# NVlabs/nvbio

Measured on NVIDIA H100. Metric: Mreads/s (150bp) seed+extend, higher is better.
Workload: dtype int32

## Files before the change

### nvbio_b200/csrc/pipeline.cu

```cuda
#include "fm_core.cuh"
#include "gotoh_core.cuh"
#include "pipeline_core.cuh"
#include "gotoh_full_core.cuh"
#include <cub/agent/single_pass_scan_operators.cuh>
#include <cub/block/block_scan.cuh>
#include <cub/device/device_scan.cuh>
#include <cub/device/device_segmented_sort.cuh>
#include <mutex>

namespace nvb {

struct PipeGeom {
    uint32_t n_reads;
    uint32_t n_strings;
    uint32_t strands;
    uint32_t stride;
    uint32_t bits;
    uint32_t seeds_per_string;
    uint32_t seed_len, seed_interval;
    uint32_t band;
    uint32_t max_seed_hits;
    uint32_t genome_len;
};

template <int BITS>
__global__ void __launch_bounds__(256)
pipe_make_strings_kernel(const StrSet reads, const PipeGeom g, uint32_t* __restrict__ out_words, uint32_t* __restrict__ out_len)
{
    constexpr uint32_t SPW = 32 / BITS;
    const uint32_t words_per_string = g.stride / SPW;
    const uint64_t t = (uint64_t)blockIdx.x * 256 + threadIdx.x;
    if (t >= (uint64_t)g.n_strings * words_per_string) return;
    const uint32_t s = (uint32_t)(t / words_per_string), w = (uint32_t)(t % words_per_string);
    const uint32_t read = s / g.strands, strand = s % g.strands;
    const uint32_t off = str_off(reads, read), len = str_len(reads, read);
    if (w == 0) out_len[s] = len;
    uint32_t word = 0;
    for (uint32_t k = 0; k < SPW; ++k) {
        const uint32_t p = w * SPW + k;
        uint32_t c = 0;
        if (p < len) {
            if (strand == 0) c = sym_at_rt(reads.words, reads.bits, reads.big_endian, off + p);
            else { c = sym_at_rt(reads.words, reads.bits, reads.big_endian, off + (len - 1u - p)); c = (c < 4u) ? 3u - c : c; }
        }
        word |= c << (32u - BITS - BITS * k);
    }
    out_words[t] = word;
}

__global__ void __launch_bounds__(256)
pipe_make_quals_kernel(const StrSet reads, const PipeGeom g, const uint8_t* __restrict__ quals, uint8_t* __restrict__ out)
{
    const uint64_t t = (uint64_t)blockIdx.x * 256 + threadIdx.x;
    if (t >= (uint64_t)g.n_strings * g.stride) return;
    const uint32_t s = (uint32_t)(t / g.stride), p = (uint32_t)(t % g.stride);
    const uint32_t read = s / g.strands, strand = s % g.strands;
// ... 130 lines not shown
        ranges[q] = make_uint2(x, y);
        if (sizes) sizes[q] = seed_range_hits(make_uint2(x, y), g.max_seed_hits);
    }
}

__device__ __forceinline__ uint32_t upper_bound_u32(const uint32_t* __restrict__ a, uint32_t n, uint32_t v)
{
    uint32_t lo = 0, hi = n;
    while (lo < hi) { const uint32_t mid = (lo + hi) >> 1; if (a[mid] <= v) lo = mid + 1; else hi = mid; }
    return lo;
}

__global__ void pipe_count_kernel(const uint32_t* __restrict__ excl, const uint32_t* __restrict__ sizes, uint32_t n_queries, uint32_t capacity,
                                  uint32_t* __restrict__ counts)
{
    if (threadIdx.x == 0 && blockIdx.x == 0) {
        const uint32_t total = n_queries ? excl[n_queries - 1] + sizes[n_queries - 1] : 0u;
        counts[1] = total;
        counts[0] = total < capacity ? total : capacity;
    }
}

__global__ void __launch_bounds__(256)
pipe_expand_hits_kernel(const FmIndex f, const PipeGeom g, const uint2* __restrict__ ranges, const uint32_t* __restrict__ sizes,
                        const uint32_t* __restrict__ excl, const uint32_t* __restrict__ slen, const uint32_t* __restrict__ counts,
                        uint32_t* __restrict__ hit_string, uint32_t* __restrict__ p_off, uint32_t* __restrict__ p_len,
                        uint32_t* __restrict__ t_off, uint32_t* __restrict__ t_len)
{
    const uint32_t q = blockIdx.x * 256 + threadIdx.x;
    if (q >= g.n_strings * g.seeds_per_string) return;
    const uint32_t sz = sizes[q];
    if (sz == 0) return;
    const uint32_t base = excl[q], kept = counts[0];
    const uint32_t x = ranges[q].x;
    const uint32_t s = q / g.seeds_per_string, k = q % g.seeds_per_string;
    const uint32_t seed_begin = k * g.seed_interval;
    const uint32_t len = slen[s];
    for (uint32_t j = 0; j < sz; ++j) {
        const uint32_t h = base + j;
        if (h >= kept) break;
        const uint2 w = hit_window(fm_locate_one(f, x + j), seed_begin, len, g);
        hit_string[h] = s;
        p_off[h] = s * g.stride; p_len[h] = len;
        t_off[h] = w.x;          t_len[h] = w.y - w.x;
    }
}

struct Jobs { uint32_t *p_off, *p_len, *t_off, *t_len; };

constexpr uint32_t RJ_BLOCK = 128;
constexpr uint32_t RJ_STAGE = 640;
constexpr int      RJ_LOCAL = 6;
constexpr uint32_t RJ_CLAIMED = 0xFFFFFFFFu, RJ_CLAIMED_EMPTY = 0xFFFFFFFEu;
using RjTileState = cub::ScanTileState<uint32_t>;
using RjPrefixOp  = cub::TilePrefixCallbackOp<uint32_t, ::cuda::std::plus<uint32_t>, RjTileState>;

__global__ void __launch_bounds__(256)
pipe_resolve_init_kernel(RjTileState tiles, const uint32_t n_tiles, uint32_t* __restrict__ counts, uint32_t* __restrict__ dp_count)
{
    tiles.InitializeStatus((int)n_tiles);
    if (blockIdx.x == 0 && threadIdx.x == 0) { counts[2] = 0u; counts[3] = 0u; *dp_count = 0u; }
}

__global__ void __launch_bounds__(RJ_BLOCK, 8)
pipe_resolve_reads_kernel(const FmIndex f, const PipeGeom g, const uint2* __restrict__ ranges, const uint32_t* __restrict__ slen,
                          const uint32_t hit_capacity, RjTileState tiles, const uint32_t n_tiles, uint32_t* __restrict__ counts,
                          const int shortcut, const int32_t match, const int32_t mismatch, const int32_t max_gap_open,
                          const uint32_t* __restrict__ str_words, const uint32_t* __restrict__ genome,
                          uint32_t* __restrict__ j_string, uint32_t* __restrict__ j_first, const Jobs jobs,
                          int32_t* __restrict__ job_score, uint2* __restrict__ job_sink,
                          const Jobs dp, uint32_t* __restrict__ dp_job, uint32_t* __restrict__ dp_count,
                          unsigned long long* __restrict__ best_key, int32_t* best_score, uint32_t* best_pos, uint8_t* __restrict__ best_strand)
{
    using BlockScan = cub::BlockScan<uint32_t, RJ_BLOCK>;
    __shared__ struct { typename RjPrefixOp::TempStorage prefix; typename BlockScan::TempStorage scan; } s_tmp;
    __shared__ uint32_t st_string[RJ_STAGE], st_first[RJ_STAGE], st_toff[RJ_STAGE], st_tlen[RJ_STAGE], st_slot[RJ_STAGE];
    __shared__ unsigned long long s_key[RJ_BLOCK];
    __shared__ int32_t s_score[RJ_BLOCK];
    __shared__ uint32_t s_pos[RJ_BLOCK];
    __shared__ uint8_t s_strand[RJ_BLOCK];
    __shared__ uint32_t s_tile, s_cnt, s_base, s_dp_cnt, s_dp_base;
    if (threadIdx.x == 0) { s_tile = atomicAdd(counts + 3, 1u); s_cnt = 0u; s_dp_cnt = 0u; }
    s_key[threadIdx.x] = 0ull;
    __syncthreads();
    const uint32_t tile = s_tile, r0 = tile * RJ_BLOCK, r = r0 + threadIdx.x;
    const uint32_t per_read = g.strands * g.seeds_per_string;
    const bool live = r < g.n_reads;
    const uint2* rr = ranges + (size_t)r * per_read;

    uint32_t hits = 0, run = 0;
    if (live)
        for (uint32_t q = 0; q < per_read; ++q) hits += seed_range_hits(rr[q], g.max_seed_hits);
    if (tile == 0) {
        uint32_t aggregate;
        BlockScan(s_tmp.scan).ExclusiveSum(hits, run, aggregate);
        if (threadIdx.x == 0) tiles.SetInclusive(0, aggregate);
    } else {
        RjPrefixOp prefix(tiles, s_tmp.prefix, ::cuda::std::plus<uint32_t>{}, (int)tile);
        BlockScan(s_tmp.scan).ExclusiveSum(hits, run, prefix);
    }
    if (tile == n_tiles - 1u && threadIdx.x == RJ_BLOCK - 1u) {
        const uint32_t total = run + hits;
        counts[1] = total;
        counts[0] = total < hit_capacity ? total : hit_capacity;
    }

    if (live) {
        uint32_t lk_s[RJ_LOCAL], lk_b[RJ_LOCAL], lk_e[RJ_LOCAL];
        int n_local = 0;
        for (uint32_t strand = 0; strand < g.strands; ++strand) {
            const uint32_t s = r * g.strands + strand;
            const uint32_t len = slen[s];
            for (uint32_t k = 0; k < g.seeds_per_string; ++k) {
                const uint2 rq = rr[strand * g.seeds_per_string + k];
                const bool located = rq.y == 0xFFFFFFFFu;
                const uint32_t sz = seed_range_hits(rq, g.max_seed_hits);
                if (sz == 0u) continue;
                const uint32_t base = run, x = rq.x, seed_begin = k * g.seed_interval;
                run += sz;
                for (uint32_t j = 0; j < sz; ++j) {
                    const uint32_t h = base + j;
                    if (h >= hit_capacity) break;
                    const uint2 w = hit_window(located ? x : fm_locate_one(f, x + j), seed_begin, len, g);
                    bool seen = false;
#pragma unroll
                    for (int e = 0; e < RJ_LOCAL; ++e) seen |= (e < n_local) && lk_s[e] == s && lk_b[e] == w.x && lk_e[e] == w.y;
                    if (seen) continue;
#pragma unroll
                    for (int e = 0; e < RJ_LOCAL; ++e) if (e == n_local) { lk_s[e] = s; lk_b[e] = w.x; lk_e[e] = w.y; }
                    if (n_local < RJ_LOCAL) ++n_local;
                    const uint32_t slot = atomicAdd(&s_cnt, 1u);
                    if (slot < RJ_STAGE) { st_string[slot] = s; st_first[slot] = h; st_toff[slot] = w.x; st_tlen[slot] = w.y - w.x; }
                    else {
                        const uint32_t o = atomicAdd(counts + 2, 1u), d = atomicAdd(dp_count, 1u);
                        j_string[o] = s; j_first[o] = h;
                        jobs.p_off[o] = s * g.stride; jobs.p_len[o] = len; jobs.t_off[o] = w.x; jobs.t_len[o] = w.y - w.x;
                        dp.p_off[d] = s * g.stride; dp.p_len[d] = len; dp.t_off[d] = w.x; dp.t_len[d] = w.y - w.x; dp_job[d] = o;
                    }
                }
            }
        }
    }
    __syncthreads();

    const uint32_t n = s_cnt < RJ_STAGE ? s_cnt : RJ_STAGE;
    if (threadIdx.x == 0) s_base = n ? atomicAdd(counts + 2, n) : 0u;
    __syncthreads();
    for (uint32_t i = threadIdx.x; i < n; i += RJ_BLOCK) {
        const uint32_t o = s_base + i, s = st_string[i], first = st_first[i], len = slen[s], to = st_toff[i], N = st_tlen[i];
        j_string[o] = s; j_first[o] = first; jobs.p_off[o] = s * g.stride; jobs.p_len[o] = len; jobs.t_off[o] = to; jobs.t_len[o] = N;
        int32_t score = 0; uint32_t sx = 0, sy = 0;
        if (shortcut && gapless_job_shortcut(str_words, genome, s * g.stride, len, to, N, g.band, match, mismatch, max_gap_open, score, sx, sy,
                                             shortcut != 2)) {
            const uint2 sk = make_uint2(sx, sy);
            job_score[o] = score; job_sink[o] = sk;
            if (job_aligned(sk)) {
                st_slot[i] = RJ_CLAIMED; st_toff[i] = to + sx; st_tlen[i] = (uint32_t)score;
                atomicMax(&s_key[s / g.strands - r0], make_best_key(score, first));
            } else st_slot[i] = RJ_CLAIMED_EMPTY;
        } else st_slot[i] = atomicAdd(&s_dp_cnt, 1u);
    }
    __syncthreads();
    if (threadIdx.x == 0) s_dp_base = s_dp_cnt ? atomicAdd(dp_count, s_dp_cnt) : 0u;
    __syncthreads();
    for (uint32_t i = threadIdx.x; i < n; i += RJ_BLOCK) {
        const uint32_t slot = st_slot[i], s = st_string[i];
        if (slot == RJ_CLAIMED) {
            const uint32_t rl = s / g.strands - r0;
            const int32_t score = (int32_t)st_tlen[i];
            if (s_key[rl] == make_best_key(score, st_first[i])) { s_score[rl] = score; s_pos[rl] = st_toff[i]; s_strand[rl] = (uint8_t)(s % g.strands); }
        } else if (slot != RJ_CLAIMED_EMPTY) {
            const uint32_t d = s_dp_base + slot;
            dp.p_off[d] = s * g.stride; dp.p_len[d] = slen[s]; dp.t_off[d] = st_toff[i]; dp.t_len[d] = st_tlen[i]; dp_job[d] = s_base + i;
        }
    }
    __syncthreads();
    if (live) {
        const unsigned long long key = s_key[threadIdx.x];
        best_key[r] = key;
        best_score[r] = key ? s_score[threadIdx.x] : INT_MIN;
        best_pos[r] = key ? s_pos[threadIdx.x] : 0xFFFFFFFFu;
        best_strand[r] = key ? s_strand[threadIdx.x] : (uint8_t)0;
    }
}

__global__ void __launch_bounds__(256)
pipe_scatter_dp_kernel(const PipeGeom g, const uint32_t* __restrict__ dp_count, const uint32_t* __restrict__ dp_job,
                       const int32_t* __restrict__ dp_score, const uint2* __restrict__ dp_sink,
                       const uint32_t* __restrict__ j_string, const uint32_t* __restrict__ j_first,
                       int32_t* __restrict__ job_score, uint2* __restrict__ job_sink, unsigned long long* __restrict__ best_key)
{
    const uint32_t n = *dp_count;
    for (uint32_t a = blockIdx.x * 256 + threadIdx.x; a < n; a += gridDim.x * 256) {
        const uint32_t j = dp_job[a];
        const int32_t sc = dp_score[a];
        const uint2 sk = dp_sink[a];
        job_score[j] = sc; job_sink[j] = sk;
        if (job_aligned(sk)) atomicMax(best_key + j_string[j] / g.strands, make_best_key(sc, j_first[j]));
    }
}

__global__ void __launch_bounds__(256)
pipe_finalize_dp_kernel(const PipeGeom g, const uint32_t* __restrict__ dp_count, const uint32_t* __restrict__ dp_job,
                        const int32_t* __restrict__ dp_score, const uint2* __restrict__ dp_sink, const uint32_t* __restrict__ dp_t_off,
                        const uint32_t* __restrict__ j_string, const uint32_t* __restrict__ j_first,
                        const unsigned long long* __restrict__ best_key,
// ... 898 lines not shown
    if (nq64 > 0x7FFFFFFFull) return NVB_E_UNSUPPORTED;
    if (nq64 * (uint64_t)P->max_seed_hits > 0xFFFFFFFFull) return NVB_E_UNSUPPORTED;

    const cudaStream_t s = c.s = as_stream(stream);
    c.P = P; c.f = make_fmindex(fmi); c.rd = make_strset(reads); c.genome = d_genome; c.nq = (uint32_t)nq64; c.hit_capacity = hit_capacity;
    c.best_score = d_best_score; c.best_pos = d_best_pos; c.hit_score = d_hit_score; c.hit_sink = d_hit_sink; c.BA = BA; c.PP = PP; c.PO = PO; c.MP = MP; c.MO = MO;
    if (PMO) {
        c.PMO = PMO;
        c.se_mo.d_second_score = PMO->d_mate_second_score; c.se_mo.d_mapq = PMO->d_mate_mapq;
        c.MO = &c.se_mo;
    }
    c.dedup = P->dedup_jobs != 0;
    c.per_read = c.dedup && g_pipe_path != 1 && !d_hit_read && !d_hit_window && !d_hit_score && !d_hit_sink;
    const nvb_gotoh_scheme& SC = P->scheme;
    c.eligible = c.per_read && P->type == NVB_LOCAL && g.bits == 2 && P->band_len <= 32 && !SC.d_qual_table && SC.match > 0 && SC.mismatch < 0 &&
                 SC.pattern_gap_open < 0 && SC.pattern_gap_ext <= 0 && SC.text_gap_open < 0 && SC.text_gap_ext <= 0;
    c.seed_split = c.per_read && c.f.sa_shift == 0u && c.f.ktab_k && g.seed_len > c.f.ktab_k && g_seed_split;
    size_t need = 0;
    NVB_TRY(c.carve(d_temp, need));
    if (!d_temp || *temp_bytes < need) { *temp_bytes = need; return NVB_E_TEMP_SIZE; }
    if (n_reads == 0) return NVB_OK;

    NVB_TRY(default_stage_events(&c.SE));
    NVB_TRY(c.stage(0));
    NVB_TRY(c.make_strings()); NVB_TRY(c.stage(1));
    NVB_TRY(c.match_seeds());  NVB_TRY(c.stage(2));
    if (!c.per_read) {
        size_t scan_bytes = c.scan_bytes;
        NVB_CUDA_TRY(cub::DeviceScan::ExclusiveSum(c.scan_tmp, scan_bytes, c.sizes, c.excl, (int)c.nq, s));
        pipe_count_kernel<<<1, 32, 0, s>>>(c.excl, c.sizes, c.nq, hit_capacity, c.counts);
        NVB_LAUNCH_CHECK();
    }
    NVB_TRY(c.stage(3));
    NVB_TRY(c.per_read ? c.extend_per_read() : c.extend_per_hit());
    if (hit_capacity && (d_hit_read || d_hit_window)) {
        pipe_export_hits_kernel<<<(hit_capacity + 255) / 256, 256, 0, s>>>(g, c.counts, c.hit_string, c.hits.t_off, c.hits.t_len, d_hit_read, (uint2*)d_hit_window);
        NVB_LAUNCH_CHECK();
    }
    if (BA && !PP) NVB_TRY(c.best_traceback());
    if (c.MO) NVB_TRY(c.second_best());
    if (PMO) NVB_TRY(c.pair_candidates());
    if (PP) NVB_TRY(c.paired_rescue());
    if (BA && PP) { NVB_TRY(c.best_traceback()); NVB_TRY(c.rescue_traceback()); }
    if (PMO) NVB_TRY(c.pair_second());
    if (!c.dedup) NVB_CUDA_TRY(cudaMemcpyAsync(c.counts + 2, c.counts, sizeof(uint32_t), cudaMemcpyDeviceToDevice, s));
    if (d_n_hits) NVB_CUDA_TRY(cudaMemcpyAsync(d_n_hits, c.counts, 3 * sizeof(uint32_t), cudaMemcpyDeviceToDevice, s));
    NVB_TRY(c.stage(7));
    c.SE->valid = true;
    return NVB_OK;
}

extern "C" void nvb_debug_pipeline_path(int path) { g_pipe_path = path; }
extern "C" void nvb_debug_seed_split(int on) { g_seed_split = on; }
extern "C" void nvb_debug_perfect_shortcut(int on) { g_perfect_shortcut = on; }
extern "C" int nvb_debug_dp_jobs(uint32_t* n)
{
    if (!n || !g_last_dp_count) return NVB_E_INVALID;
    NVB_CUDA_TRY(cudaDeviceSynchronize());
    NVB_CUDA_TRY(cudaMemcpy(n, g_last_dp_count, sizeof(uint32_t), cudaMemcpyDeviceToHost));
    return NVB_OK;
}

extern "C" int nvb_seed_extend(const nvb_fm_index* fmi, const uint32_t* d_genome,
                    const nvb_string_set* reads, uint32_t n_reads,
                    const nvb_seed_extend_params* P, uint32_t hit_capacity,
                    int32_t* d_best_score, uint32_t* d_best_pos,
                    uint32_t* d_n_hits, uint32_t* d_hit_read, nvb_uint2* d_hit_window,
                    int32_t* d_hit_score, nvb_uint2* d_hit_sink,
                    void* d_temp, size_t* temp_bytes, void* stream)
{
    return seed_extend_impl(fmi, d_genome, reads, n_reads, P, hit_capacity, d_best_score, d_best_pos, d_n_hits, d_hit_read, d_hit_window,
                            d_hit_score, d_hit_sink, nullptr, nullptr, nullptr, nullptr, nullptr, nullptr, d_temp, temp_bytes, stream);
}

extern "C" int nvb_seed_extend_traceback(const nvb_fm_index* fmi, const uint32_t* d_genome,
                    const nvb_string_set* reads, uint32_t n_reads,
                    const nvb_seed_extend_params* P, uint32_t hit_capacity,
                    int32_t* d_best_score, uint32_t* d_best_pos,
                    uint32_t* d_n_hits, uint32_t* d_hit_read, nvb_uint2* d_hit_window,
                    int32_t* d_hit_score, nvb_uint2* d_hit_sink,
                    const nvb_best_alignment_out* best_alignment,
                    void* d_temp, size_t* temp_bytes, void* stream)
{
    if (!best_alignment) return NVB_E_INVALID;
    return seed_extend_impl(fmi, d_genome, reads, n_reads, P, hit_capacity, d_best_score, d_best_pos, d_n_hits, d_hit_read, d_hit_window,
                            d_hit_score, d_hit_sink, best_alignment, nullptr, nullptr, nullptr, nullptr, nullptr, d_temp, temp_bytes, stream);
}

extern "C" int nvb_seed_extend_paired(const nvb_fm_index* fmi, const uint32_t* d_genome,
                    const nvb_string_set* reads, uint32_t n_pairs,
                    const nvb_seed_extend_params* P, uint32_t hit_capacity,
                    const nvb_pair_params* pair_params, const nvb_pair_out* out,
                    uint32_t* d_n_hits, void* d_temp, size_t* temp_bytes, void* stream)
{
    if (!pair_params || !out || n_pairs > 0x3FFFFFFFu || !temp_bytes) return NVB_E_INVALID;
    return seed_extend_impl(fmi, d_genome, reads, 2u * n_pairs, P, hit_capacity, out->d_mate_score, out->d_mate_pos, d_n_hits, nullptr, nullptr,
                            nullptr, nullptr, nullptr, pair_params, out, nullptr, nullptr, nullptr, d_temp, temp_bytes, stream);
}

extern "C" int nvb_seed_extend_mapq(const nvb_fm_index* fmi, const uint32_t* d_genome,
                    const nvb_string_set* reads, uint32_t n_reads,
                    const nvb_seed_extend_params* P, uint32_t hit_capacity,
                    int32_t* d_best_score, uint32_t* d_best_pos,
                    uint32_t* d_n_hits, uint32_t* d_hit_read, nvb_uint2* d_hit_window,
                    int32_t* d_hit_score, nvb_uint2* d_hit_sink,
                    const nvb_best_alignment_out* best_alignment,
                    const nvb_mapq_params* mapq, const nvb_mapq_out* mapq_out,
// ... 52 lines not shown
```

### nvbio_b200/csrc/pipeline_core.cuh

```cuda
#pragma once
#include "fm_core.cuh"

namespace nvb {

__host__ __device__ __forceinline__ uint32_t nvb_clz(uint32_t x) {
#ifdef __CUDA_ARCH__
    return (uint32_t)__clz((int)x);
#else
    return (uint32_t)__builtin_clz(x);
#endif
}

__host__ __device__ __forceinline__ uint32_t job_diff_bits(const uint32_t* __restrict__ str_words, const uint32_t* __restrict__ genome,
                                                           const uint32_t po, const uint32_t t, const uint32_t i, const uint32_t cnt)
{
    const uint32_t x = (be2_window(str_words, po + i, cnt) ^ be2_window(genome, t + i, cnt)) >> (32u - 2u * cnt);
    return (x | (x >> 1)) & 0x55555555u;
}
__host__ __device__ __forceinline__ uint32_t job_differences(const uint32_t* __restrict__ str_words, const uint32_t* __restrict__ genome,
                                                             const uint32_t po, const uint32_t M, const uint32_t t, const uint32_t limit)
{
    uint32_t mm = 0;
    for (uint32_t i = 0; i < M && mm <= limit; i += 16u) mm += nvb_popc(job_diff_bits(str_words, genome, po, t, i, M - i < 16u ? M - i : 16u));
    return mm;
}

__host__ __device__ __forceinline__ uint32_t diff_row_mask(const uint32_t w0, const uint32_t cnt, const uint32_t lo, const uint32_t hi)
{
    const uint32_t a = lo > w0 ? lo : w0, b = hi < w0 + cnt - 1u ? hi : w0 + cnt - 1u;
    if (a > b) return 0u;
    return ((2u << (2u * (w0 + cnt - 1u - a))) - 1u) & ~((1u << (2u * (w0 + cnt - 1u - b))) - 1u);
}
__host__ __device__ inline void job_diff_span(const uint32_t* __restrict__ str_words, const uint32_t* __restrict__ genome, const uint32_t po,
                                              const uint32_t t, const uint32_t lo, const uint32_t hi, int32_t& first, int32_t& last)
{
    first = (int32_t)hi + 1; last = (int32_t)lo - 1;
    for (uint32_t i = lo; i <= hi; i += 16u) {
        const uint32_t cnt = hi + 1u - i < 16u ? hi + 1u - i : 16u;
        const uint32_t d = job_diff_bits(str_words, genome, po, t, i, cnt);
        if (!d) continue;
        if (first > (int32_t)hi) first = (int32_t)(i + cnt - 1u - ((31u - nvb_clz(d)) >> 1));
        last = (int32_t)(i + cnt - 1u - ((31u - nvb_clz(d & (0u - d))) >> 1));
    }
}
__host__ __device__ __forceinline__ uint32_t text_window16(const uint32_t g0, const uint32_t g1, const uint32_t g2, const uint32_t g3, const uint32_t off)
{
    const uint32_t idx = off >> 4, sh = 2u * (off & 15u);
    const uint32_t hi = idx == 0u ? g0 : (idx == 1u ? g1 : g2), lo = idx == 0u ? g1 : (idx == 1u ? g2 : g3);
    return sh ? ((hi << sh) | (lo >> (32u - sh))) : hi;
}

__host__ __device__ inline bool gapless_job_shortcut(const uint32_t* __restrict__ str_words, const uint32_t* __restrict__ genome,
                                                     const uint32_t po, const uint32_t M, const uint32_t to, const uint32_t N, const uint32_t band,
                                                     const int32_t match, const int32_t mismatch, const int32_t max_gap_open,
                                                     int32_t& score, uint32_t& sink_x, uint32_t& sink_y, const bool one_gap = true)
{
    if (M < 1u || to == 0u || N < M + band - 1u) return false;
    const uint32_t j0 = band / 2u;
    const int32_t o = -max_gap_open, lim = !one_gap ? o : (o + match - mismatch < 2 * o ? o + match - mismatch : 2 * o);
    const uint32_t mm_max = (uint32_t)((lim - 1) / match);
    int32_t h = 0, best = 0, f1 = (int32_t)M, f2 = (int32_t)M, l1 = -1, l2 = -1; uint32_t end = 0, prev = 0, mm0 = 0;
    for (uint32_t i = 0; i < M && mm0 <= mm_max; i += 16u) {
        const uint32_t cnt = M - i < 16u ? M - i : 16u;
        uint32_t d = job_diff_bits(str_words, genome, po, to + j0, i, cnt);
        while (d && mm0 <= mm_max) {
            const uint32_t bit = 31u - nvb_clz(d);
            const uint32_t p = i + (cnt - 1u - (bit >> 1));
            d &= ~(1u << bit);
            h += match * (int32_t)(p - prev);
            if (h >= best) { best = h; end = p; }
            h += mismatch; h = h > 0 ? h : 0;
            if (mm0 == 0u) f1 = (int32_t)p; else if (mm0 == 1u) f2 = (int32_t)p;
            l2 = l1; l1 = (int32_t)p;
            prev = p + 1u; ++mm0;
        }
    }
    if (mm0 > mm_max) return false;
    h += match * (int32_t)(M - prev);
    if (h >= best) { best = h; end = M; }
    const int32_t delta = match * (int32_t)M - best;
    if (delta >= lim) return false;
    const bool gap1 = delta >= o;
    const uint32_t U = gap1 ? (uint32_t)((delta - o) / match) : 0u;
    if (gap1 && 2u * U + 1u > M) return false;
    const uint32_t hi = M - 1u - U;
    int32_t fa = f1 >= (int32_t)U ? f1 : (f2 >= (int32_t)U ? f2 : (int32_t)(M - U)), ba = l1 <= (int32_t)hi ? l1 : (l2 <= (int32_t)hi ? l2 : (int32_t)U - 1);
    fa = fa > (int32_t)hi ? (int32_t)(M - U) : fa; ba = ba < (int32_t)U ? (int32_t)U - 1 : ba;
    int32_t fb = INT_MIN, bb = INT_MAX; uint32_t fd = j0, bd = j0;
    const bool perfect = (mm0 == 0u);
    const uint32_t t = (uint32_t)(delta / match);
    const uint32_t c16 = M < 16u ? M : 16u;
    const uint32_t r0 = be2_window(str_words, po, c16) >> (32u - 2u * c16);
    const uint32_t wi = to >> 4, r = to & 15u, wl = (to + N - 1u) >> 4;
    const uint32_t g0 = genome[wi], g1 = (wi + 1u <= wl) ? genome[wi + 1u] : 0u;
    const uint32_t g2 = (wi + 2u <= wl) ? genome[wi + 2u] : 0u, g3 = (wi + 3u <= wl) ? genome[wi + 3u] : 0u;
    uint32_t rE = 0, e0 = 0, e1 = 0, e2 = 0, e3 = 0, mF = 0, mB = 0;
    const uint32_t te = to + M - c16, we = te >> 4;
    if (gap1) {
        rE = be2_window(str_words, po + M - c16, c16) >> (32u - 2u * c16);
        e0 = genome[we]; e1 = (we + 1u <= wl) ? genome[we + 1u] : 0u; e2 = (we + 2u <= wl) ? genome[we + 2u] : 0u; e3 = (we + 3u <= wl) ? genome[we + 3u] : 0u;
        mF = diff_row_mask(0u, c16, U, hi); mB = diff_row_mask(M - c16, c16, U, hi);
    }
    uint32_t jtop = j0;
    for (uint32_t jj = 0; jj < band; ++jj) {
        if (jj == j0) continue;
        const uint32_t x = (text_window16(g0, g1, g2, g3, r + jj) >> (32u - 2u * c16)) ^ r0, dx = (x | (x >> 1)) & 0x55555555u;
        if (gap1) {
            const uint32_t y = (text_window16(e0, e1, e2, e3, (te & 15u) + jj) >> (32u - 2u * c16)) ^ rE, dy = (y | (y >> 1)) & 0x55555555u & mB;
            int32_t F, B;
            if ((dx & mF) && dy) { F = (int32_t)(c16 - 1u - ((31u - nvb_clz(dx & mF)) >> 1)); B = (int32_t)(M - 1u - ((31u - nvb_clz(dy & (0u - dy))) >> 1)); }
            else job_diff_span(str_words, genome, po, to + jj, U, hi, F, B);
            if (F > fa) { fb = fa; fa = F; fd = jj; } else if (F > fb) fb = F;
            if (B < ba) { bb = ba; ba = B; bd = jj; } else if (B < bb) bb = B;
        }
        if (nvb_popc(dx) > t) continue;
        if (job_differences(str_words, genome, po, M, to + jj, t) > t) continue;
        if (!perfect) return false;
        if (jj > jtop) jtop = jj;
    }
    if (gap1 && (fd != bd ? (int64_t)ba - fa : ((int64_t)ba - fb < (int64_t)bb - fa ? (int64_t)ba - fb : (int64_t)bb - fa)) <= (int64_t)U - 1) return false;
    score = best;
    if (perfect) { sink_x = M + jtop; sink_y = M; }
    else         { sink_x = end + j0; sink_y = end; }
    return true;
}

__host__ __device__ __forceinline__ bool distinct_alignment(uint32_t p, uint32_t t, uint32_t bp, uint32_t bt, uint32_t len)
{
    const uint32_t d = len / 2u;
    return t != bt || p < bp - (bp < d ? bp : d) || p > bp + d;
}

__host__ __device__ __forceinline__ uint32_t aln_begin(uint32_t end, uint32_t len) { return end > len ? end - len : 0u; }

__host__ __device__ __forceinline__ bool fr_concordant(uint32_t fb, uint32_t fe, uint32_t rb, uint32_t re, uint32_t min_frag, uint32_t max_frag)
{
    return fb <= rb && fe <= re && re > fb && (re - fb) >= min_frag && (re - fb) <= max_frag;
}

struct PairSecond {
    uint32_t star_end[2], star_strand[2], len[2];
    bool has; int32_t score; uint32_t end[2], strand[2], tie[2];

    __host__ __device__ __forceinline__ void init(uint32_t e1, uint32_t t1, uint32_t l1, uint32_t e2, uint32_t t2, uint32_t l2)
    {
        star_end[0] = e1; star_strand[0] = t1; len[0] = l1; star_end[1] = e2; star_strand[1] = t2; len[1] = l2;
        has = false; score = INT_MIN; end[0] = end[1] = 0xFFFFFFFFu; strand[0] = strand[1] = 0u; tie[0] = tie[1] = 0xFFFFFFFFu;
    }
    __host__ __device__ __forceinline__ void offer(int32_t s, uint32_t e1, uint32_t t1, uint32_t i1, uint32_t e2, uint32_t t2, uint32_t i2)
    {
        if (!distinct_alignment(e1, t1, star_end[0], star_strand[0], len[0]) && !distinct_alignment(e2, t2, star_end[1], star_strand[1], len[1]))
            return;
        if (has && (s < score || (s == score && (i1 > tie[0] || (i1 == tie[0] && i2 >= tie[1]))))) return;
        has = true; score = s; end[0] = e1; strand[0] = t1; tie[0] = i1; end[1] = e2; strand[1] = t2; tie[1] = i2;
    }
    __host__ __device__ __forceinline__ void offer_rescue(int a, int32_t s, uint32_t ae, uint32_t at, uint32_t ai, uint32_t oe)
    {
        if (a == 0) offer(s, ae, at, ai, oe, 1u - at, 0xFFFFFFFFu);
        else        offer(s, oe, 1u - at, 0xFFFFFFFFu, ae, at, ai);
    }
};

struct MateCands { const uint32_t* end; const int32_t* score; const uint32_t* tie; uint32_t n_fw, n, len; };

__host__ __device__ __forceinline__ uint32_t lower_bound_end(const uint32_t* end, uint32_t lo, uint32_t hi, uint64_t v)
{
    while (lo < hi) { const uint32_t mid = (lo + hi) >> 1; if ((uint64_t)end[mid] < v) lo = mid + 1; else hi = mid; }
    return lo;
}

__host__ __device__ inline void pair_combinations(const MateCands m[2], uint32_t min_frag, uint32_t max_frag, PairSecond& ps)
{
    for (int a = 0; a < 2; ++a) {
// ... 82 lines not shown
```

### nvbio_b200/csrc/fm_core.cuh

```cuda
#pragma once
#include "common.cuh"

namespace nvb {

struct __align__(32) FmBlock {
    uint32_t bwt[4];
    uint32_t occ[4];
};

struct FmIndex {
    const FmBlock*  blocks;
    const uint32_t* ssa;
    const uint2*    ktab;
    uint32_t n, primary;
    uint32_t L2[5];
    uint32_t sa_mask, sa_shift;
    uint32_t ktab_k;
    uint32_t ktab_located;
    const uint2*    rows;
    uint32_t ktab_wide;
    __host__ __device__ __forceinline__ uint32_t l2(uint32_t c) const {
        return (c == 0) ? L2[0] : (c == 1) ? L2[1] : (c == 2) ? L2[2] : L2[3];
    }
    __host__ __device__ __forceinline__ uint32_t count(uint32_t c) const {
// ... 136 lines not shown
    const uint32_t m = r / SPW;
    const uint64_t off = k * (K / SPW);
    I out = occ[k * 4u + c];
    for (uint32_t j = 0; j < m; ++j) out += word_rank<W>(text[off + j], c, SPW);
    return out + word_rank<W>(text[off + m], c, (r % SPW) + 1u);
}

__host__ __device__ __forceinline__ uint32_t fm_rank1(const FmIndex& f, uint32_t k, uint32_t c) {
    if (k == 0xFFFFFFFFu) return 0u;
    if (k == f.n) return f.count(c);
    if (k >= f.primary) --k;
    const FmBlock b = load_block(f.blocks, k >> 6);
    return block_rank(b, k & 63u, c);
}

__host__ __device__ __forceinline__ uint4 fm_rank4(const FmIndex& f, uint32_t k) {
    if (k == 0xFFFFFFFFu) return make_uint4(0u, 0u, 0u, 0u);
    if (k == f.n) return make_uint4(f.count(0), f.count(1), f.count(2), f.count(3));
    if (k >= f.primary) --k;
    const FmBlock b = load_block(f.blocks, k >> 6);
    const uint32_t r = k & 63u;
    return make_uint4(block_rank(b, r, 0), block_rank(b, r, 1), block_rank(b, r, 2), block_rank(b, r, 3));
}

__host__ __device__ __forceinline__ void fm_rank2(const FmIndex& f, uint32_t kx, uint32_t ky, uint32_t c,
                                                  uint32_t& rx, uint32_t& ry) {
    const bool need_x = (kx != 0xFFFFFFFFu) && (kx != f.n);
    const bool need_y = (ky != 0xFFFFFFFFu) && (ky != f.n);
    const uint32_t cnt = f.count(c);
    rx = (kx == f.n) ? cnt : 0u;
    ry = (ky == f.n) ? cnt : 0u;
    const uint32_t ax = kx - (kx >= f.primary ? 1u : 0u);
    const uint32_t ay = ky - (ky >= f.primary ? 1u : 0u);
    if (need_x || need_y) {
        const uint32_t bx = ax >> 6, by = ay >> 6;
        FmBlock b0 = load_block(f.blocks, need_x ? bx : by);
        FmBlock b1 = b0;
        load_block_if(b1, f.blocks, by, need_x && need_y && bx != by);
        const uint32_t tx = block_rank(b0, ax & 63u, c);
        const uint32_t ty = block_rank(b1, ay & 63u, c);
        if (need_x) rx = tx;
        if (need_y) ry = ty;
    }
}

__host__ __device__ __forceinline__ void fm_step(const FmIndex& f, uint32_t c, uint32_t& x, uint32_t& y) {
    uint32_t rx, ry;
    fm_rank2(f, x - 1u, y, c, rx, ry);
    const uint32_t base = f.l2(c);
    x = base + rx + 1u;
    y = base + ry;
}

__host__ __device__ __forceinline__ uint32_t be2_window(const uint32_t* __restrict__ words, uint32_t a, uint32_t cnt)
{
    const uint32_t wi = a >> 4, r = a & 15u;
    const uint32_t w0 = words[wi];
    if (r == 0u) return w0;
    const uint32_t w1 = (r + cnt > 16u) ? words[wi + 1u] : 0u;
    return (w0 << (2u * r)) | (w1 >> (32u - 2u * r));
}

constexpr uint32_t KTAB_TWO_ROW_MARK = 0xC0000000u;
__host__ __device__ __forceinline__ bool ktab_two_row_marker(const FmIndex& f, const uint32_t y) {
    return f.ktab_located == 2u && f.n < KTAB_TWO_ROW_MARK && y >= KTAB_TWO_ROW_MARK;
}

__host__ __device__ __forceinline__ uint32_t text_before(const uint32_t* __restrict__ text, const uint32_t pos, const uint32_t want)
{
    const uint32_t cnt = (pos == 0xFFFFFFFFu) ? 0u : (pos < want ? pos : want);
    return cnt ? (be2_window(text, pos - cnt, cnt) >> (32u - 2u * cnt)) : 0u;
}

constexpr uint32_t KTAB_WIDE_ROWS = 8;
__host__ __device__ __forceinline__ void ktab_wide_fill(const uint32_t* __restrict__ sa, const uint32_t* __restrict__ text, uint32_t n,
                                                        uint32_t x, uint32_t y, uint32_t (&w)[8])
{
#pragma unroll
    for (int i = 0; i < 8; ++i) w[i] = 0u;
    w[0] = x; w[1] = y;
    if (x > y) return;
    const uint32_t d = y - x;
    if (d == 0u) { w[2] = sa[x]; w[3] = text_before(text, w[2], 16u); return; }
    if (d == 1u) {
        w[2] = sa[x]; w[3] = sa[y];
        if (n < KTAB_TWO_ROW_MARK) w[1] = KTAB_TWO_ROW_MARK | text_before(text, w[2], 7u) | (text_before(text, w[3], 7u) << 14);
        return;
    }
    if (d == 2u) {
#pragma unroll
        for (int i = 0; i < 3; ++i) { w[2 + i] = sa[x + i]; w[5 + i] = text_before(text, w[2 + i], 16u); }
        return;
    }
    if (d >= KTAB_WIDE_ROWS) return;
#pragma unroll
    for (uint32_t i = 0; i < KTAB_WIDE_ROWS; ++i) {
        if (i > d) continue;
        const uint32_t pos = sa[x + i];
        w[2 + i / 2u] |= text_before(text, pos, 8u) << (16u * (i & 1u));
        if (d == 3u) w[4 + i] = pos;
    }
}
__host__ __device__ __forceinline__ uint32_t ktab_wide_context(const uint4& lo, const uint4& hi, bool three, uint32_t i)
{
    if (three) return i == 0u ? hi.y : (i == 1u ? hi.z : hi.w);
    const uint32_t w = i < 2u ? lo.z : (i < 4u ? lo.w : (i < 6u ? hi.x : hi.y));
    return (i & 1u) ? (w >> 16) : (w & 0xFFFFu);
// ... 328 lines not shown
```

Baseline: 399.4.

## Extend gapless shortcut to a deeper tier proving optimality for more mismatches

Adds a third tier to the gapless-alignment shortcut so that a job with a larger score deficit (up to two gap opens or gap plus mismatches) can still be resolved without full DP. The extra per-diagonal checks and a final middle-window scan rule out alternative gapped alignments. The default shortcut mode now uses this deeper tier, so more jobs skip the Gotoh DP stage. The cost is more work per job in the shortcut path and a risk of incorrect optimality proofs.

```diff
diff --git a/nvbio_b200/csrc/pipeline.cu b/nvbio_b200/csrc/pipeline.cu
--- a/nvbio_b200/csrc/pipeline.cu
+++ b/nvbio_b200/csrc/pipeline.cu
@@ -337,7 +337,7 @@
         j_string[o] = s; j_first[o] = first; jobs.p_off[o] = s * g.stride; jobs.p_len[o] = len; jobs.t_off[o] = to; jobs.t_len[o] = N;
         int32_t score = 0; uint32_t sx = 0, sy = 0;
         if (shortcut && gapless_job_shortcut(str_words, genome, s * g.stride, len, to, N, g.band, match, mismatch, max_gap_open, score, sx, sy,
-                                             shortcut != 2)) {
+                                             shortcut == 1 ? 2 : (shortcut == 3 ? 1 : 0))) {
             const uint2 sk = make_uint2(sx, sy);
             job_score[o] = score; job_sink[o] = sk;
             if (job_aligned(sk)) {
@@ -1342,7 +1342,7 @@
 
 extern "C" void nvb_debug_pipeline_path(int path) { g_pipe_path = path; }
 extern "C" void nvb_debug_seed_split(int on) { g_seed_split = on; }
-extern "C" void nvb_debug_perfect_shortcut(int on) { g_perfect_shortcut = on; }
+extern "C" void nvb_debug_perfect_shortcut(int on) { g_perfect_shortcut = (on >= 0 && on <= 3) ? on : 1; }
 extern "C" int nvb_debug_dp_jobs(uint32_t* n)
 {
     if (!n || !g_last_dp_count) return NVB_E_INVALID;
diff --git a/nvbio_b200/csrc/pipeline_core.cuh b/nvbio_b200/csrc/pipeline_core.cuh
--- a/nvbio_b200/csrc/pipeline_core.cuh
+++ b/nvbio_b200/csrc/pipeline_core.cuh
@@ -53,11 +53,13 @@
 __host__ __device__ inline bool gapless_job_shortcut(const uint32_t* __restrict__ str_words, const uint32_t* __restrict__ genome,
                                                      const uint32_t po, const uint32_t M, const uint32_t to, const uint32_t N, const uint32_t band,
                                                      const int32_t match, const int32_t mismatch, const int32_t max_gap_open,
-                                                     int32_t& score, uint32_t& sink_x, uint32_t& sink_y, const bool one_gap = true)
+                                                     int32_t& score, uint32_t& sink_x, uint32_t& sink_y, const int tier = 2)
 {
     if (M < 1u || to == 0u || N < M + band - 1u) return false;
     const uint32_t j0 = band / 2u;
-    const int32_t o = -max_gap_open, lim = !one_gap ? o : (o + match - mismatch < 2 * o ? o + match - mismatch : 2 * o);
+    const int32_t o = -max_gap_open, ms = match - mismatch;
+    const int32_t lim1 = o + ms < 2 * o ? o + ms : 2 * o, lim2 = 3 * o < 2 * o + ms ? (3 * o < o + 2 * ms ? 3 * o : o + 2 * ms) : (2 * o + ms < o + 2 * ms ? 2 * o + ms : o + 2 * ms);
+    const int32_t lim = tier == 0 ? o : (tier == 1 ? lim1 : lim2);
     const uint32_t mm_max = (uint32_t)((lim - 1) / match);
     int32_t h = 0, best = 0, f1 = (int32_t)M, f2 = (int32_t)M, l1 = -1, l2 = -1; uint32_t end = 0, prev = 0, mm0 = 0;
     for (uint32_t i = 0; i < M && mm0 <= mm_max; i += 16u) {
@@ -80,16 +82,39 @@
     if (h >= best) { best = h; end = M; }
     const int32_t delta = match * (int32_t)M - best;
     if (delta >= lim) return false;
-    const bool gap1 = delta >= o;
+    const bool gap1 = delta >= o, deep = delta >= lim1;
     const uint32_t U = gap1 ? (uint32_t)((delta - o) / match) : 0u;
     if (gap1 && 2u * U + 1u > M) return false;
     const uint32_t hi = M - 1u - U;
     int32_t fa = f1 >= (int32_t)U ? f1 : (f2 >= (int32_t)U ? f2 : (int32_t)(M - U)), ba = l1 <= (int32_t)hi ? l1 : (l2 <= (int32_t)hi ? l2 : (int32_t)U - 1);
     fa = fa > (int32_t)hi ? (int32_t)(M - U) : fa; ba = ba < (int32_t)U ? (int32_t)U - 1 : ba;
+    const uint32_t c16 = M < 16u ? M : 16u;
+    uint32_t q2 = 0u;
+    if (deep) {
+        if (mm0 > 4u || M > 0xFFFFu) return false;
+        uint32_t xa = 0u, kb = 15u, lo3 = 0u, cm = 0u;
+        if (delta >= o + ms) {
+            const int32_t c3 = mm0 == 3u ? l1 : (mm0 == 4u ? l2 : (int32_t)M), c4 = mm0 == 4u ? l1 : (int32_t)M;
+            const int32_t d3 = mm0 == 3u ? f1 : (mm0 == 4u ? f2 : -1), d4 = mm0 == 4u ? f1 : -1;
+            const int32_t F2j = f1 >= (int32_t)U ? f2 : (f2 >= (int32_t)U ? c3 : (c3 >= (int32_t)U ? c4 : (int32_t)M));
+            const int32_t B2j = l1 <= (int32_t)hi ? l2 : (l2 <= (int32_t)hi ? d3 : (d3 <= (int32_t)hi ? d4 : -1));
+            const int32_t U2 = (delta - o - ms) / match, tB = B2j - U2, kF = (int32_t)M - 1 - (F2j + U2);
+            if (tB < 0 || kF < 0 || (int32_t)M - 2 * (int32_t)c16 + 1 < U2) return false;
+            if (tB < (int32_t)c16 - 1) xa = c16 - 1u - (uint32_t)tB;
+            if (kF < 15) kb = (uint32_t)kF;
+        }
+        if (delta >= 2 * o) {
+            const int32_t U3 = (delta - 2 * o) / match;
+            const int32_t a3 = (fa > (int32_t)c16 - 1 ? fa : (int32_t)c16 - 1) + U3, hi3 = (ba < (int32_t)(M - c16) ? ba : (int32_t)(M - c16)) - U3;
+            if (a3 > hi3) return false;
+            if (!((f1 >= a3 && f1 <= hi3) || (f2 >= a3 && f2 <= hi3) || (l2 >= a3 && l2 <= hi3) || (l1 >= a3 && l1 <= hi3))) return false;
+            lo3 = (uint32_t)a3; cm = hi3 - a3 + 1 < 16 ? (uint32_t)(hi3 - a3 + 1) : 16u;
+        }
+        q2 = cm | (xa << 5) | (kb << 9) | (1u << 13) | (lo3 << 16);
+    }
     int32_t fb = INT_MIN, bb = INT_MAX; uint32_t fd = j0, bd = j0;
     const bool perfect = (mm0 == 0u);
     const uint32_t t = (uint32_t)(delta / match);
-    const uint32_t c16 = M < 16u ? M : 16u;
     const uint32_t r0 = be2_window(str_words, po, c16) >> (32u - 2u * c16);
     const uint32_t wi = to >> 4, r = to & 15u, wl = (to + N - 1u) >> 4;
     const uint32_t g0 = genome[wi], g1 = (wi + 1u <= wl) ? genome[wi + 1u] : 0u;
@@ -112,6 +137,10 @@
             else job_diff_span(str_words, genome, po, to + jj, U, hi, F, B);
             if (F > fa) { fb = fa; fa = F; fd = jj; } else if (F > fb) fb = F;
             if (B < ba) { bb = ba; ba = B; bd = jj; } else if (B < bb) bb = B;
+            if (q2 & (1u << 13)) {
+                const uint32_t v = dx & mF, a = v ? v ^ (0x80000000u >> nvb_clz(v)) : 0u, b = dy & (dy - 1u);
+                if (a < (1u << (2u * ((q2 >> 5) & 15u))) || !(b & ((4u << (2u * ((q2 >> 9) & 15u))) - 1u))) q2 |= 1u << 14;
+            }
         }
         if (nvb_popc(dx) > t) continue;
         if (job_differences(str_words, genome, po, M, to + jj, t) > t) continue;
@@ -119,6 +148,15 @@
         if (jj > jtop) jtop = jj;
     }
     if (gap1 && (fd != bd ? (int64_t)ba - fa : ((int64_t)ba - fb < (int64_t)bb - fa ? (int64_t)ba - fb : (int64_t)bb - fa)) <= (int64_t)U - 1) return false;
+    if (q2 & (1u << 14)) return false;
+    if (q2 & 31u) {
+        const uint32_t lo3 = q2 >> 16, cm = q2 & 31u;
+        const uint32_t rm = be2_window(str_words, po + lo3, cm) >> (32u - 2u * cm), tm = to + lo3, wm = tm >> 4;
+        const uint32_t m0 = genome[wm], m1 = (wm + 1u <= wl) ? genome[wm + 1u] : 0u;
+        const uint32_t m2 = (wm + 2u <= wl) ? genome[wm + 2u] : 0u, m3 = (wm + 3u <= wl) ? genome[wm + 3u] : 0u;
+        for (uint32_t jj = 0; jj < band; ++jj)
+            if (jj != j0 && (text_window16(m0, m1, m2, m3, (tm & 15u) + jj) >> (32u - 2u * cm)) == rm) return false;
+    }
     score = best;
     if (perfect) { sink_x = M + jtop; sink_y = M; }
     else         { sink_x = end + j0; sink_y = end; }
```

Measured after the change: 399.0 (median of 6 runs). About the same (-0.1%).

## Vectorize seed-range scan per warp and stage shortcut words in shared memory

Applied to the files above, without the earlier changes.

The resolve kernel now reads seed ranges cooperatively per warp with 16-byte vector loads, building per-read hit counts and a nonzero-seed bitmask in shared memory through atomics. The per-read loop then visits only seeds whose bit is set, prefetching several ranges ahead. For the gapless shortcut, read and genome words are copied into a strided shared-memory buffer with cp.async before scoring, and the DP helpers are templated so they can read from that buffer. The aim is to cut scattered, uncoalesced global loads, at the cost of extra shared memory (which may reduce occupancy), shared atomics and more code complexity.

```diff
diff --git a/nvbio_b200/csrc/fm_core.cuh b/nvbio_b200/csrc/fm_core.cuh
--- a/nvbio_b200/csrc/fm_core.cuh
+++ b/nvbio_b200/csrc/fm_core.cuh
@@ -212,7 +212,8 @@
     y = base + ry;
 }
 
-__host__ __device__ __forceinline__ uint32_t be2_window(const uint32_t* __restrict__ words, uint32_t a, uint32_t cnt)
+template <class Words>
+__host__ __device__ __forceinline__ uint32_t be2_window(const Words words, uint32_t a, uint32_t cnt)
 {
     const uint32_t wi = a >> 4, r = a & 15u;
     const uint32_t w0 = words[wi];
diff --git a/nvbio_b200/csrc/pipeline.cu b/nvbio_b200/csrc/pipeline.cu
--- a/nvbio_b200/csrc/pipeline.cu
+++ b/nvbio_b200/csrc/pipeline.cu
@@ -2,6 +2,7 @@
 #include "gotoh_core.cuh"
 #include "pipeline_core.cuh"
 #include "gotoh_full_core.cuh"
+#include <cuda_pipeline.h>
 #include <cub/agent/single_pass_scan_operators.cuh>
 #include <cub/block/block_scan.cuh>
 #include <cub/device/device_scan.cuh>
@@ -238,6 +239,9 @@
 constexpr uint32_t RJ_STAGE = 640;
 constexpr int      RJ_LOCAL = 6;
 constexpr uint32_t RJ_CLAIMED = 0xFFFFFFFFu, RJ_CLAIMED_EMPTY = 0xFFFFFFFEu;
+constexpr int      RJ_VEC = 7;
+constexpr int      RJ_AHEAD = 4;
+constexpr uint32_t RJ_WORDS = 23;
 using RjTileState = cub::ScanTileState<uint32_t>;
 using RjPrefixOp  = cub::TilePrefixCallbackOp<uint32_t, ::cuda::std::plus<uint32_t>, RjTileState>;
 
@@ -266,6 +270,7 @@
     __shared__ uint32_t s_pos[RJ_BLOCK];
     __shared__ uint8_t s_strand[RJ_BLOCK];
     __shared__ uint32_t s_tile, s_cnt, s_base, s_dp_cnt, s_dp_base;
+    __shared__ union { struct { uint32_t hits[RJ_BLOCK], mask[RJ_BLOCK]; } a; uint32_t words[RJ_WORDS * RJ_BLOCK]; } s_u;
     if (threadIdx.x == 0) { s_tile = atomicAdd(counts + 3, 1u); s_cnt = 0u; s_dp_cnt = 0u; }
     s_key[threadIdx.x] = 0ull;
     __syncthreads();
@@ -274,8 +279,41 @@
     const bool live = r < g.n_reads;
     const uint2* rr = ranges + (size_t)r * per_read;
 
+    const bool masked = per_read <= 32u && ((size_t)ranges & 15u) == 0u;
     uint32_t hits = 0, run = 0;
-    if (live)
+    if (masked) {
+        const uint32_t lane = threadIdx.x & 31u, w0 = threadIdx.x & ~31u, wr0 = r0 + w0;
+        s_u.a.hits[threadIdx.x] = 0u; s_u.a.mask[threadIdx.x] = 0u;
+        __syncwarp();
+        const uint32_t nq = wr0 < g.n_reads ? (g.n_reads - wr0 < 32u ? g.n_reads - wr0 : 32u) * per_read : 0u;
+        const uint2* wb = ranges + (size_t)wr0 * per_read;
+        for (uint32_t v0 = 0; 2u * v0 < nq; v0 += 32u * RJ_VEC) {
+            uint4 v[RJ_VEC];
+#pragma unroll
+            for (int b = 0; b < RJ_VEC; ++b) {
+                const uint32_t q = 2u * (v0 + b * 32u + lane);
+                if (q + 1u < nq) v[b] = reinterpret_cast<const uint4*>(wb)[q >> 1];
+                else { const uint2 t = q < nq ? wb[q] : make_uint2(1u, 0u); v[b] = make_uint4(t.x, t.y, 1u, 0u); }
+            }
+#pragma unroll
+            for (int b = 0; b < RJ_VEC; ++b) {
+                const uint32_t q = 2u * (v0 + b * 32u + lane), rd = q / per_read, k = q - rd * per_read;
+                const uint32_t sz0 = seed_range_hits(make_uint2(v[b].x, v[b].y), g.max_seed_hits);
+                const uint32_t sz1 = seed_range_hits(make_uint2(v[b].z, v[b].w), g.max_seed_hits);
+                if (k + 1u < per_read) {
+                    if (sz0 | sz1) {
+                        atomicAdd(&s_u.a.hits[w0 + rd], sz0 + sz1);
+                        atomicOr(&s_u.a.mask[w0 + rd], (sz0 ? 1u << k : 0u) | (sz1 ? 2u << k : 0u));
+                    }
+                } else {
+                    if (sz0) { atomicAdd(&s_u.a.hits[w0 + rd], sz0); atomicOr(&s_u.a.mask[w0 + rd], 1u << k); }
+                    if (sz1) { atomicAdd(&s_u.a.hits[w0 + rd + 1u], sz1); atomicOr(&s_u.a.mask[w0 + rd + 1u], 1u); }
+                }
+            }
+        }
+        __syncwarp();
+        hits = s_u.a.hits[threadIdx.x];
+    } else if (live)
         for (uint32_t q = 0; q < per_read; ++q) hits += seed_range_hits(rr[q], g.max_seed_hits);
     if (tile == 0) {
         uint32_t aggregate;
@@ -294,38 +332,51 @@
     if (live) {
         uint32_t lk_s[RJ_LOCAL], lk_b[RJ_LOCAL], lk_e[RJ_LOCAL];
         int n_local = 0;
-        for (uint32_t strand = 0; strand < g.strands; ++strand) {
+        const uint32_t len0 = slen[r * g.strands], len1 = g.strands > 1u ? slen[r * g.strands + 1u] : 0u;
+        auto take = [&](const uint32_t q, const uint2 rq) {
+            const uint32_t strand = q / g.seeds_per_string, k = q - strand * g.seeds_per_string;
             const uint32_t s = r * g.strands + strand;
-            const uint32_t len = slen[s];
-            for (uint32_t k = 0; k < g.seeds_per_string; ++k) {
-                const uint2 rq = rr[strand * g.seeds_per_string + k];
-                const bool located = rq.y == 0xFFFFFFFFu;
-                const uint32_t sz = seed_range_hits(rq, g.max_seed_hits);
-                if (sz == 0u) continue;
-                const uint32_t base = run, x = rq.x, seed_begin = k * g.seed_interval;
-                run += sz;
-                for (uint32_t j = 0; j < sz; ++j) {
-                    const uint32_t h = base + j;
-                    if (h >= hit_capacity) break;
-                    const uint2 w = hit_window(located ? x : fm_locate_one(f, x + j), seed_begin, len, g);
-                    bool seen = false;
+            const bool located = rq.y == 0xFFFFFFFFu;
+            const uint32_t sz = seed_range_hits(rq, g.max_seed_hits);
+            if (sz == 0u) return;
+            const uint32_t len = strand ? len1 : len0;
+            const uint32_t base = run, x = rq.x, seed_begin = k * g.seed_interval;
+            run += sz;
+            for (uint32_t j = 0; j < sz; ++j) {
+                const uint32_t h = base + j;
+                if (h >= hit_capacity) break;
+                const uint2 w = hit_window(located ? x : fm_locate_one(f, x + j), seed_begin, len, g);
+                bool seen = false;
 #pragma unroll
-                    for (int e = 0; e < RJ_LOCAL; ++e) seen |= (e < n_local) && lk_s[e] == s && lk_b[e] == w.x && lk_e[e] == w.y;
-                    if (seen) continue;
+                for (int e = 0; e < RJ_LOCAL; ++e) seen |= (e < n_local) && lk_s[e] == s && lk_b[e] == w.x && lk_e[e] == w.y;
+                if (seen) continue;
 #pragma unroll
-                    for (int e = 0; e < RJ_LOCAL; ++e) if (e == n_local) { lk_s[e] = s; lk_b[e] = w.x; lk_e[e] = w.y; }
-                    if (n_local < RJ_LOCAL) ++n_local;
-                    const uint32_t slot = atomicAdd(&s_cnt, 1u);
-                    if (slot < RJ_STAGE) { st_string[slot] = s; st_first[slot] = h; st_toff[slot] = w.x; st_tlen[slot] = w.y - w.x; }
-                    else {
-                        const uint32_t o = atomicAdd(counts + 2, 1u), d = atomicAdd(dp_count, 1u);
-                        j_string[o] = s; j_first[o] = h;
-                        jobs.p_off[o] = s * g.stride; jobs.p_len[o] = len; jobs.t_off[o] = w.x; jobs.t_len[o] = w.y - w.x;
-                        dp.p_off[d] = s * g.stride; dp.p_len[d] = len; dp.t_off[d] = w.x; dp.t_len[d] = w.y - w.x; dp_job[d] = o;
-                    }
+                for (int e = 0; e < RJ_LOCAL; ++e) if (e == n_local) { lk_s[e] = s; lk_b[e] = w.x; lk_e[e] = w.y; }
+                if (n_local < RJ_LOCAL) ++n_local;
+                const uint32_t slot = atomicAdd(&s_cnt, 1u);
+                if (slot < RJ_STAGE) { st_string[slot] = s; st_first[slot] = h; st_toff[slot] = w.x; st_tlen[slot] = w.y - w.x; }
+                else {
+                    const uint32_t o = atomicAdd(counts + 2, 1u), d = atomicAdd(dp_count, 1u);
+                    j_string[o] = s; j_first[o] = h;
+                    jobs.p_off[o] = s * g.stride; jobs.p_len[o] = len; jobs.t_off[o] = w.x; jobs.t_len[o] = w.y - w.x;
+                    dp.p_off[d] = s * g.stride; dp.p_len[d] = len; dp.t_off[d] = w.x; dp.t_len[d] = w.y - w.x; dp_job[d] = o;
                 }
             }
-        }
+        };
+        if (masked) {
+            for (uint32_t m = s_u.a.mask[threadIdx.x]; m; ) {
+                uint2 rq[RJ_AHEAD]; uint32_t qs[RJ_AHEAD];
+#pragma unroll
+                for (int b = 0; b < RJ_AHEAD; ++b) {
+                    qs[b] = m ? (uint32_t)__ffs((int)m) - 1u : 32u;
+                    if (m) rq[b] = rr[qs[b]];
+                    m &= m - 1u;
+                }
+#pragma unroll
+                for (int b = 0; b < RJ_AHEAD; ++b) if (qs[b] < 32u) take(qs[b], rq[b]);
+            }
+        } else
+            for (uint32_t q = 0; q < per_read; ++q) take(q, rr[q]);
     }
     __syncthreads();
 
@@ -336,8 +387,21 @@
         const uint32_t o = s_base + i, s = st_string[i], first = st_first[i], len = slen[s], to = st_toff[i], N = st_tlen[i];
         j_string[o] = s; j_first[o] = first; jobs.p_off[o] = s * g.stride; jobs.p_len[o] = len; jobs.t_off[o] = to; jobs.t_len[o] = N;
         int32_t score = 0; uint32_t sx = 0, sy = 0;
-        if (shortcut && gapless_job_shortcut(str_words, genome, s * g.stride, len, to, N, g.band, match, mismatch, max_gap_open, score, sx, sy,
-                                             shortcut != 2)) {
+        bool claimed = false;
+        if (shortcut) {
+            const uint32_t po = s * g.stride, nr = (len + 15u) >> 4, wi = to >> 4, nw = N ? ((to + N - 1u) >> 4) - wi + 1u : 0u;
+            if (nr + nw <= RJ_WORDS) {
+                uint32_t* b = s_u.words + threadIdx.x;
+                for (uint32_t k = 0; k < nr; ++k) __pipeline_memcpy_async(b + k * RJ_BLOCK, str_words + (po >> 4) + k, 4);
+                for (uint32_t k = 0; k < nw; ++k) __pipeline_memcpy_async(b + (nr + k) * RJ_BLOCK, genome + wi + k, 4);
+                __pipeline_commit();
+                __pipeline_wait_prior(0);
+                claimed = gapless_job_shortcut(StagedWords{b, po >> 4, RJ_BLOCK}, StagedWords{b + nr * RJ_BLOCK, wi, RJ_BLOCK}, po, len, to, N,
+                                               g.band, match, mismatch, max_gap_open, score, sx, sy, shortcut != 2);
+            } else
+                claimed = gapless_job_shortcut(str_words, genome, po, len, to, N, g.band, match, mismatch, max_gap_open, score, sx, sy, shortcut != 2);
+        }
+        if (claimed) {
             const uint2 sk = make_uint2(sx, sy);
             job_score[o] = score; job_sink[o] = sk;
             if (job_aligned(sk)) {
diff --git a/nvbio_b200/csrc/pipeline_core.cuh b/nvbio_b200/csrc/pipeline_core.cuh
--- a/nvbio_b200/csrc/pipeline_core.cuh
+++ b/nvbio_b200/csrc/pipeline_core.cuh
@@ -11,13 +11,20 @@
 #endif
 }
 
-__host__ __device__ __forceinline__ uint32_t job_diff_bits(const uint32_t* __restrict__ str_words, const uint32_t* __restrict__ genome,
+struct StagedWords {
+    const uint32_t* p; uint32_t base, stride;
+    __host__ __device__ __forceinline__ uint32_t operator[](const uint32_t i) const { return p[(i - base) * stride]; }
+};
+
+template <class W>
+__host__ __device__ __forceinline__ uint32_t job_diff_bits(const W str_words, const W genome,
                                                            const uint32_t po, const uint32_t t, const uint32_t i, const uint32_t cnt)
 {
     const uint32_t x = (be2_window(str_words, po + i, cnt) ^ be2_window(genome, t + i, cnt)) >> (32u - 2u * cnt);
     return (x | (x >> 1)) & 0x55555555u;
 }
-__host__ __device__ __forceinline__ uint32_t job_differences(const uint32_t* __restrict__ str_words, const uint32_t* __restrict__ genome,
+template <class W>
+__host__ __device__ __forceinline__ uint32_t job_differences(const W str_words, const W genome,
                                                              const uint32_t po, const uint32_t M, const uint32_t t, const uint32_t limit)
 {
     uint32_t mm = 0;
@@ -31,7 +38,8 @@
     if (a > b) return 0u;
     return ((2u << (2u * (w0 + cnt - 1u - a))) - 1u) & ~((1u << (2u * (w0 + cnt - 1u - b))) - 1u);
 }
-__host__ __device__ inline void job_diff_span(const uint32_t* __restrict__ str_words, const uint32_t* __restrict__ genome, const uint32_t po,
+template <class W>
+__host__ __device__ inline void job_diff_span(const W str_words, const W genome, const uint32_t po,
                                               const uint32_t t, const uint32_t lo, const uint32_t hi, int32_t& first, int32_t& last)
 {
     first = (int32_t)hi + 1; last = (int32_t)lo - 1;
@@ -50,7 +58,8 @@
     return sh ? ((hi << sh) | (lo >> (32u - sh))) : hi;
 }
 
-__host__ __device__ inline bool gapless_job_shortcut(const uint32_t* __restrict__ str_words, const uint32_t* __restrict__ genome,
+template <class W>
+__host__ __device__ inline bool gapless_job_shortcut(const W str_words, const W genome,
                                                      const uint32_t po, const uint32_t M, const uint32_t to, const uint32_t N, const uint32_t band,
                                                      const int32_t match, const int32_t mismatch, const int32_t max_gap_open,
                                                      int32_t& score, uint32_t& sink_x, uint32_t& sink_y, const bool one_gap = true)
```

After: 400.3 before, 404.5 after (median of 6 runs). 1.01x the previous value.
